# pyranha-labs/hypergrep

Measured on AMD Instinct MI355X. Metric: GiB/s scanned (256 patterns, 32 GiB synthetic log per GPU, text resident in HBM), higher is better.
Workload: dtype u8

## Files before the change

hypergrep_amd/build.py:

```python
from __future__ import annotations

import os
import shutil
import subprocess
import sys

PKG = os.path.dirname(os.path.abspath(__file__))
REPO = os.path.dirname(PKG)
CSRC = os.path.join(PKG, "csrc")
LIB_DIR = os.path.join(PKG, "lib")
LIB = os.path.join(LIB_DIR, "libhyperscanner.so")
LIBHS_NAME = "libhs.so.5"
OBJ = os.path.join(REPO, "build", "obj")
EXTRA = os.environ.get("HG_BUILD_DEFINES", "").split()
if os.environ.get("HG_BUILD_OUT"):
    LIB = os.path.abspath(os.environ["HG_BUILD_OUT"])
    LIB_DIR = os.path.dirname(LIB)
    OBJ = LIB + ".obj"
    LIBHS_NAME = os.path.basename(LIB) + ".libhs.so.5"

HIP_SOURCES = ["hg_stream.hip", "hg_kernels.hip", "hg_always_on.hip", "hg_huge.hip", "hg_som.hip", "hg_comb.hip", "hg_invert.hip", "hg_flows.hip", "hg_batch.hip", "hg_engine.hip", "hg_capi.hip", "hg_shim.hip", "hg_hsface.hip"]
CXX_SOURCES = ["hg_compile.cpp"]
HEADERS = ["hg_mem.h", "hg_db.h", "hg_core.h", "hg_post.h", "hg_engine.h", "hg_compile.h", "hg_synth.h", "hg_confirm_dev.h", "hg_sink_dev.h", "hg_tables_dev.h", "hg_som.h", "hg_comb.h", "hg_invert.h", "hg_flows.h", "hg_flow_rules.h", "hg_batch.h", "hg_batch_launch.h"]

# ... 44 lines not shown

def _merge_resources() -> None:
    import json

    table = {}
    for src in KERNEL_SOURCES:
        path = os.path.join(OBJ, src + ".resources.json")
        if os.path.exists(path):
            with open(path, encoding="utf-8") as f:
                table.update(json.load(f))
    with open(os.path.join(LIB_DIR, "kernel_resources.json"), "w", encoding="utf-8") as f:
        json.dump(table, f, indent=1, sort_keys=True)
    for kernel, res in table.items():
        if kernel.startswith("_Z16hg_stream_kernelILi") and "ELb0ELi0E" in kernel and res.get("ScratchSize [bytes/lane]", 0) > 16:
            raise RuntimeError(f"{kernel} uses {res['ScratchSize [bytes/lane]']} bytes of scratch per lane: the streaming hot path must stay in registers")
        if "hg_som_kernel" in kernel and res.get("ScratchSize [bytes/lane]", 0) > 0:
            raise RuntimeError(f"{kernel} uses {res['ScratchSize [bytes/lane]']} bytes of scratch per lane: the start-of-match walks keep their state in registers / LDS")
        if "hg_minlen_kernel" in kernel and res.get("ScratchSize [bytes/lane]", 0) > 0:
            raise RuntimeError(f"{kernel} uses {res['ScratchSize [bytes/lane]']} bytes of scratch per lane: the match-length walks keep their state in registers / LDS")
        if "hg_flow_som_kernel" in kernel and res.get("ScratchSize [bytes/lane]", 0) > 0:
            raise RuntimeError(f"{kernel} uses {res['ScratchSize [bytes/lane]']} bytes of scratch per lane: the stream-mode start-of-match lanes keep their starts in device memory")
        if "hg_block_batch_kernel" in kernel and (res.get("ScratchSize [bytes/lane]", 0) > 0 or res.get("VGPRs Spill", 0) > 0):
            raise RuntimeError(f"{kernel} uses {res['ScratchSize [bytes/lane]']} bytes of scratch per lane, {res['VGPRs Spill']} spilled VGPRs: the batched block scan keeps its automaton state in registers")
        if "hg_comb_kernel" in kernel and res.get("ScratchSize [bytes/lane]", 0) > 0:
            raise RuntimeError(f"{kernel} uses {res['ScratchSize [bytes/lane]']} bytes of scratch per lane: the combination pass keeps its evaluation stack in a register")


def build(verbose: bool = False, force: bool = False) -> str:
    from concurrent.futures import ThreadPoolExecutor

    os.makedirs(OBJ, exist_ok=True)
    os.makedirs(LIB_DIR, exist_ok=True)
    hipcc = _hipcc()
    common_deps = [os.path.join(CSRC, h) for h in HEADERS] + [os.path.join(REPO, "include", "hypergrep_amd.h")]
    objs, jobs = [], []
    for src in HIP_SOURCES + CXX_SOURCES:
        path = os.path.join(CSRC, src)
        if not os.path.exists(path):
            continue
        obj = os.path.join(OBJ, src + ".o")
        objs.append(obj)
        if force or _stale(obj, [path] + common_deps):
            if src.endswith(".hip"):
                cmd = [hipcc, "--offload-arch=gfx950", "-O3", "-std=c++17", "-fPIC", "-Wall", "-Wno-pass-failed"] + EXTRA + ["-c", path, "-o", obj]
            else:
                cmd = ["g++", "-O2", "-std=c++17", "-fPIC", "-Wall", "-Wextra", "-c", path, "-o", obj]
# ... 34 lines not shown
```

hypergrep_amd/csrc/hg_engine.h:

```cpp
#pragma once
#include <hip/hip_runtime.h>

#include <memory>
#include <string>

#include "../../include/hypergrep_amd.h"
#include "hg_compile.h"
#include "hg_core.h"
#include "hg_invert.h"
#include "hg_post.h"

#ifndef HG_STREAM_WG_WAVES
#define HG_STREAM_WG_WAVES 8
#endif
constexpr uint32_t HG_STREAM_WG_WAVES_DEFAULT = HG_STREAM_WG_WAVES;

constexpr uint32_t HG_CONFIRM_SPLIT = 4;
constexpr uint32_t HG_DEFER_SHARDS = 64;

struct HgDeferred {
  uint64_t pos;
  uint32_t pattern;
  uint32_t rank;
};
// ... 196 lines not shown
  HgTileElem *d_agg_ = nullptr;
  HgCand *d_cands_ = nullptr;
  HgDeferred *d_deferred_ = nullptr;
  uint32_t *d_defer_count_ = nullptr;
  HgHit *d_hits_raw_ = nullptr, *d_hits_out_ = nullptr;
  HgHitAux *d_aux_raw_ = nullptr, *d_aux_out_ = nullptr;
  HgHit *d_acc_hits_ = nullptr;
  HgHitAux *d_acc_aux_ = nullptr;
  uint64_t acc_cap_ = 0;
  bool side_bound_ = false;
  uint64_t *d_key_a_ = nullptr, *d_key_b_ = nullptr;
  uint32_t *d_perm_a_ = nullptr, *d_perm_b_ = nullptr;
  uint8_t *d_keep_ = nullptr;
  uint32_t *d_counters_ = nullptr, *d_selected_ = nullptr, *d_seg_count_ = nullptr;
  uint32_t max_segs_ = 0;
  uint32_t *d_pflags_ = nullptr;
  void *d_temp_ = nullptr;
  size_t temp_bytes_ = 0;
  uint32_t *h_counters_ = nullptr;
  HgTileBase *h_final_ = nullptr;
  hipEvent_t ev_[4] = {nullptr, nullptr, nullptr, nullptr};
  static constexpr int kMaxChunks = 64;
  hipStream_t side_stream_ = nullptr;
  hipEvent_t ev_tile_done_ = nullptr;
  hipEvent_t ev_fin_early_ = nullptr;
  hipEvent_t ev_k1_begin_[kMaxChunks] = {}, ev_k1_end_[kMaxChunks] = {}, ev_side_done_[kMaxChunks] = {};
  uint32_t *d_fin_fill_ = nullptr, *d_fin_kept_ = nullptr, *d_fin_total_ = nullptr, *d_fin_big_ = nullptr;
  bool fin_fallback_ = false;
  uint32_t fin_alloc_ = 0;
  uint32_t fin_epoch_ = 0;
  uint64_t fin_expect_hits_ = 0;
  void *d_huge_claim_ = nullptr;
  uint64_t huge_claim_slots_ = 0;
  uint32_t *d_from_ = nullptr;
  uint64_t from_cap_ = 0;
  uint32_t som_max_nw_ = 0;
  uint32_t *d_min_lengths_ = nullptr;
  HgHit *d_minlen_hits_ = nullptr;
  HgHitAux *d_minlen_aux_ = nullptr;
  uint64_t minlen_cap_ = 0;
  uint32_t minlen_max_nw_ = 0;
  HgComb *d_combs_ = nullptr;
  uint32_t *d_comb_words_ = nullptr, *d_comb_feed_ = nullptr;
  uint32_t *d_comb_count_ = nullptr;
  uint64_t *d_comb_pos_ = nullptr;
  uint64_t comb_in_cap_ = 0;
  HgHit *d_comb_hits_ = nullptr;
// ... 15 lines not shown
```

hypergrep_amd/csrc/hg_engine.hip:

```cpp
#include <algorithm>
#include <array>
#include <cstdio>
#include <cstdlib>
#include <cstring>
#include <memory>

#include "hg_engine.h"
#include "hg_mem.h"

#include <rocprim/rocprim.hpp>

bool hg_launch_stream(const HgStreamArgs &a, uint32_t grid, hipStream_t stream);
bool hg_launch_stream_join(const HgStreamArgs &a, uint32_t grid, hipStream_t stream);
int hg_stream_blocks_per_cu(uint32_t filter_log2, uint32_t filter_wide, uint32_t dense);
__global__ void hg_tile_reduce_kernel(const HgTileSum *sums, uint64_t tile_begin, uint64_t tile_end, uint64_t bs1, HgTileElem *agg);
__global__ void hg_tile_spine_kernel(const HgTileElem *agg, uint32_t nblocks, uint64_t bs1, HgTileBase *block_base, HgTileBase *state);
__global__ void hg_tile_apply_kernel(const HgTileSum *sums, uint64_t tile_begin, uint64_t tile_end, uint64_t bs1, const HgTileBase *block_base,
                                     HgTileBase *bases);
__global__ void hg_tile_inner_kernel(const uint8_t *text, HgTileSum *sums, uint64_t tile_begin, uint64_t tile_end, uint64_t bs1);
__global__ void hg_verify_kernel(HgConfirmArgs a);
__global__ void hg_confirm_fast_kernel(HgConfirmArgs a, uint32_t blocks_per_mode);
__global__ void hg_confirm_generic_kernel(HgConfirmArgs a);
__global__ void hg_always_on_kernel(HgConfirmArgs a, uint32_t first, uint32_t last);
__global__ void hg_always_on_fast_kernel(HgConfirmArgs a);
__global__ void hg_always_on_finish_kernel(HgConfirmArgs a);
__global__ void hg_block_mark_kernel(HgConfirmArgs a, uint32_t *pattern_flags);
__global__ void hg_block_scan_kernel(HgConfirmArgs a, const uint32_t *pattern_flags);
__global__ void hg_block_small_kernel(HgDbView db, const uint8_t *h_text, uint32_t length, HgHit *h_out, uint32_t seg_cap, uint32_t *h_counts, uint32_t *d_done,
                                      uint32_t *h_flag, uint32_t seq, uint32_t ppw);
__global__ void hg_reset_kernel(uint32_t *state, uint32_t state_words, HgTileBase *final_state, uint64_t carry_start, uint64_t first_piece, uint32_t *fill, uint32_t nb, uint32_t *defer_count,
                                uint32_t ndefer);
__global__ void hg_fin_sort_small_kernel(const HgHit *hits, uint32_t *idx, const uint32_t *fill, uint32_t b_lo, uint32_t b_hi, uint32_t cap, uint32_t id_bits,
                                         uint32_t to_bits, uint32_t *kept_count, uint32_t *big_list, uint32_t *big_count, uint32_t big_stride);
template <uint32_t LCAP, bool IN_LDS>
__global__ void hg_fin_sort_big_kernel(const HgHit *hits, uint32_t *idx, const uint32_t *fill, const uint32_t *big_list, const uint32_t *big_count, uint32_t cap,
                                       uint32_t id_bits, uint32_t to_bits, uint32_t *kept_count, uint32_t *overflow, uint64_t *scratch_key, uint32_t *scratch_idx);
template <uint32_t THREADS>
__global__ void hg_fin_scan_kernel(uint32_t *kept_count, uint32_t b_lo, uint32_t b_hi, uint32_t *total, const uint32_t *fill, uint32_t cap, uint32_t *part, uint32_t epoch);
__global__ void hg_confirm_literal_kernel(HgConfirmArgs a);
__global__ void hg_verify_lean_kernel(HgConfirmArgs a);
__global__ void hg_fin_gather_kernel(const HgHit *hits, const HgHitAux *aux, const uint32_t *idx, const uint32_t *kept_base, const uint32_t *total, uint32_t b_lo,
                                     uint32_t b_hi, uint32_t cap, HgHit *oh, HgHitAux *oa);
__global__ void hg_key_kernel(const HgHit *hits, const HgHitAux *aux, const HgPattern *patterns, uint32_t n, uint64_t *key, uint32_t *idx);
__global__ void hg_line_key_kernel(const HgHit *hits, const uint32_t *perm, uint32_t n, uint64_t *key);
__global__ void hg_offset_kernel(uint32_t *idx, uint32_t n, uint32_t add);
__global__ void hg_key_packed_kernel(const HgHit *hits, const HgHitAux *aux, const HgPattern *patterns, uint32_t n, uint32_t id_bits, uint32_t to_bits,
                                     uint64_t *key, uint32_t *idx);
__global__ void hg_keep_kernel(const HgHit *hits, const HgHitAux *aux, const uint32_t *perm, const HgPattern *patterns, uint32_t n, uint8_t *keep);
__global__ void hg_scatter_kernel(const HgHit *hits, const HgHitAux *aux, const uint32_t *perm, const uint8_t *keep, const uint32_t *pos, uint32_t n,
                                  HgHit *oh, HgHitAux *oa, uint32_t *count);

size_t hg_huge_lds_bytes(uint32_t nw_max, uint32_t stage_cap);
bool hg_launch_confirm_huge(const HgConfirmArgs &a, uint32_t grid, uint32_t nw_max, uint32_t stage_cap, void *claim, uint32_t claim_mask, hipStream_t stream);
bool hg_launch_always_on_huge(const HgConfirmArgs &a, uint32_t grid, uint32_t nw_max, uint32_t stage_cap, uint32_t first, uint32_t last, hipStream_t stream);
bool hg_launch_block_huge(const HgConfirmArgs &a, uint32_t grid, uint32_t nw_max, uint32_t stage_cap, const uint32_t *pattern_flags, hipStream_t stream);

namespace {
constexpr int TS_BLOCK_TILES = 1024;
constexpr int STREAM_WG_WAVES = HG_STREAM_WG_WAVES;

template <typename T>
hipError_t upload(void **dst, const std::vector<T> &src, const char *name) {
  size_t bytes = std::max<size_t>(src.size() * sizeof(T), 16);
// ... 121 lines not shown
    const HgPattern &p = db.patterns[i];
    if (p.flags & HG_FLAG_SOM_LEFTMOST) som_max_nw_ = std::max(som_max_nw_, p.nw);
    if (!db.min_lengths.empty() && db.min_lengths[i]) minlen_max_nw_ = std::max(minlen_max_nw_, p.nw);
  }
  if (db.comb_pass()) {
    HG_TRY(upload(reinterpret_cast<void **>(&d_combs_), db.combs, "d_combs_"), "upload combinations");
    HG_TRY(upload(reinterpret_cast<void **>(&d_comb_words_), db.comb_words, "d_comb_words_"), "upload combinations");
    HG_TRY(upload(reinterpret_cast<void **>(&d_comb_feed_), db.comb_feed, "d_comb_feed_"), "upload combinations");
  }
  view_.fold_mask = db.fold_mask;
  view_.window_mask = db.window_mask;
  static_assert(HG_CNT_CURSORS == kMaxChunks, "one tile cursor per pipeline chunk");
  HG_TRY(hgmem::dev_alloc(&d_counters_, HG_ST_ALLOC_WORDS * 4, "d_state_"), "alloc state");
  HG_TRY(hipMemset(d_counters_, 0, HG_ST_ALLOC_WORDS * 4), "clear state");
  d_fin_total_ = d_counters_ + HG_ST_FIN_TOTAL;
  d_selected_ = d_counters_ + HG_ST_SELECTED;
  d_final_ = reinterpret_cast<HgTileBase *>(d_counters_ + HG_ST_FINAL);
  HG_TRY(hgmem::dev_alloc(&d_pflags_, db.patterns.size() * 4 + 16, "d_pflags_"), "alloc pattern flags");
  HG_TRY(hgmem::host_alloc(&h_counters_, (HG_CNT_WORDS + 4 + HG_DEFER_SHARDS) * 4, "h_counters_"), "alloc pinned");
  h_final_ = reinterpret_cast<HgTileBase *>(h_counters_ + HG_ST_FINAL);
  for (auto &ev : ev_) HG_TRY(hipEventCreate(&ev), "hipEventCreate");
  HG_TRY(hipStreamCreateWithFlags(&side_stream_, hipStreamNonBlocking), "hipStreamCreate");
  HG_TRY(hipEventCreateWithFlags(&ev_fin_early_, hipEventDisableTiming), "hipEventCreate");
  HG_TRY(hipEventCreateWithFlags(&ev_tile_done_, hipEventDisableTiming), "hipEventCreate");
  return HG_OK;
}

HgScanner::~HgScanner() {
  (void)hipSetDevice(device_);
  void *ptrs[] = {d_patterns_, d_pool_, d_factors_, d_windows_, d_bucket_, d_filter_, d_ext_, d_slow_, d_sums_, d_bases_, d_block_base_,
                  d_agg_, d_cands_, d_hits_raw_, d_hits_out_, d_aux_raw_, d_aux_out_,
                  d_key_a_, d_key_b_, d_perm_a_, d_perm_b_, d_keep_, d_counters_, d_temp_, d_seg_count_, d_pflags_, d_deferred_, d_defer_count_, d_seg_count2_, d_cands2_, d_disc_, d_bucket2_, d_windows2_, d_groups_, d_acc_hits_, d_acc_aux_, d_huge_claim_, d_wtab_, d_from_, d_fin_fill_, d_fin_kept_, d_fin_big_,
                  d_combs_, d_comb_words_, d_comb_feed_, d_comb_count_, d_comb_pos_, d_comb_hits_, d_comb_aux_, d_comb_temp_, d_bounds_,
                  d_min_lengths_, d_minlen_hits_, d_minlen_aux_, d_inv_count_, d_inv_pos_, d_inv_temp_, d_inv_hits_, d_inv_aux_};
  for (void *p : ptrs) hgmem::dev_free(p, "scanner");
  hgmem::host_free(h_counters_, "h_counters_");
  for (auto &ev : ev_)
    if (ev) (void)hipEventDestroy(ev);
  for (int i = 0; i < kMaxChunks; i++) {
    if (ev_k1_begin_[i]) (void)hipEventDestroy(ev_k1_begin_[i]);
    if (ev_k1_end_[i]) (void)hipEventDestroy(ev_k1_end_[i]);
    if (ev_side_done_[i]) (void)hipEventDestroy(ev_side_done_[i]);
  }
  if (side_stream_) (void)hipStreamDestroy(side_stream_);
  if (ev_fin_early_) (void)hipEventDestroy(ev_fin_early_);
  if (ev_tile_done_) (void)hipEventDestroy(ev_tile_done_);
}

int HgScanner::alloc_cands(uint64_t n) {
  n = std::min<uint64_t>(n, 0x7FFFFFF0u);
  HG_TRY(realloc_dev(d_cands_, n, "d_cands_"), "workspace alloc (candidates)");
  HG_TRY(realloc_dev(d_cands2_, n, "d_cands2_"), "workspace alloc (candidates)");
  uint32_t modes = 0;
  for (uint32_t m = 0; m < HG_CONFIRM_MODES; m++) modes += db_->n_confirm_mode[m] ? 1 : 0;
  HG_TRY(realloc_dev(d_deferred_, std::max<uint64_t>(modes, 1) * n, "d_deferred_"), "workspace alloc (deferred)");
  hgmem::dev_free(d_huge_claim_, "d_huge_claim_");
  d_huge_claim_ = nullptr;
  huge_claim_slots_ = 0;
  if (db_->n_confirm_mode[4]) {
    uint64_t slots = 1u << 12;
    while (slots < 2 * n) slots <<= 1;
    HG_TRY(hgmem::dev_alloc(&d_huge_claim_, slots * 8, "d_huge_claim_"), "workspace alloc (claim table)");
    huge_claim_slots_ = slots;
  }
  cand_cap_ = static_cast<uint32_t>(n);
  return HG_OK;
}

int HgScanner::alloc_hits(uint64_t n64) {
// ... 179 lines not shown
      ca.mode_present[m] = (db_->n_confirm_mode[m] && ((mode_mask >> m) & 1u)) ? 1 : 0;
      ca.list_of_mode[m] = db_->n_confirm_mode[m] ? next++ : 0;
      ca.list_spread[m] = std::min<uint32_t>(HG_DEFER_SHARDS, std::max<uint32_t>(1, HG_DEFER_SHARDS / std::max<uint32_t>(1, db_->n_confirm_mode[m])) * defer_spread_boost_);
    }
  }
  return p;
}

int HgScanner::alloc_fin(uint32_t nb, hipStream_t stream) {
  uint32_t want = 1u << 16;
  while (want < nb) want <<= 1;
  fin_alloc_ = 0;
  HG_TRY(realloc_dev(d_fin_fill_, want, "d_fin_fill_"), "alloc finalize buckets");
  HG_TRY(realloc_dev(d_fin_kept_, want, "d_fin_kept_"), "alloc finalize buckets");
  HG_TRY(realloc_dev(d_fin_big_, 2 * static_cast<size_t>(want) + 3 * 128, "d_fin_big_"), "alloc finalize buckets");
  HG_TRY(hipMemsetAsync(d_fin_big_ + 2 * static_cast<size_t>(want), 0, 3 * 128 * 4, stream), "clear scan flags");
  fin_alloc_ = want;
  return HG_OK;
}

int HgScanner::launch_fin(const PassPlan &p, hipStream_t s, uint32_t lo, uint32_t hi, bool beside_stream) {
  if (hi <= lo) return HG_OK;
  const uint32_t nbk = hi - lo, cu = static_cast<uint32_t>(num_cus_), fin_cap = p.fin_cap, id_bits = p.id_bits, to_bits = p.to_bits;
  HG_TRY(hipMemsetAsync(d_fin_total_ + 2, 0, 8, s), "memset work list");
  hipLaunchKernelGGL(hg_fin_sort_small_kernel, dim3(std::min<uint32_t>((nbk + 3) / 4, cu * 8)), dim3(256), 0, s, d_hits_raw_, d_perm_a_, d_fin_fill_, lo, hi, fin_cap, id_bits, to_bits,
                     d_fin_kept_, d_fin_big_, d_fin_total_ + 2, fin_alloc_);
  hipLaunchKernelGGL((hg_fin_sort_big_kernel<HG_FIN_MEDIUM_CAP, true>), dim3(std::min<uint32_t>(nbk, cu * 4)), dim3(256), 0, s, d_hits_raw_, d_perm_a_, d_fin_fill_, d_fin_big_, d_fin_total_ + 2,
                     fin_cap, id_bits, to_bits, d_fin_kept_, d_selected_ + 1, static_cast<uint64_t *>(nullptr), static_cast<uint32_t *>(nullptr));
  const uint32_t big_blocks = std::min<uint32_t>(std::min<uint32_t>(nbk, 64u), hit_cap_ / HG_FIN_BUCKET_CAP);
  if (big_blocks)
    hipLaunchKernelGGL((hg_fin_sort_big_kernel<HG_FIN_BUCKET_CAP, false>), dim3(big_blocks), dim3(256), 0, s, d_hits_raw_, d_perm_a_, d_fin_fill_, d_fin_big_ + fin_alloc_,
                       d_fin_total_ + 3, fin_cap, id_bits, to_bits, d_fin_kept_, d_selected_ + 1, d_key_a_, d_perm_b_);
  const uint32_t scan_blocks = std::max<uint32_t>(1, std::min<uint32_t>(128, (nbk + 8191) / 8192));
  uint32_t *part = d_fin_big_ + 2 * static_cast<size_t>(fin_alloc_);
  const uint32_t epoch = ++fin_epoch_ ? fin_epoch_ : ++fin_epoch_;
  if (beside_stream) hipLaunchKernelGGL(hg_fin_scan_kernel<512u>, dim3(scan_blocks), dim3(512), 0, s, d_fin_kept_, lo, hi, d_fin_total_, d_fin_fill_, fin_cap, part, epoch);
  else hipLaunchKernelGGL(hg_fin_scan_kernel<1024u>, dim3(scan_blocks), dim3(1024), 0, s, d_fin_kept_, lo, hi, d_fin_total_, d_fin_fill_, fin_cap, part, epoch);
  hipLaunchKernelGGL(hg_fin_gather_kernel, dim3(std::min<uint32_t>((nbk + 3) / 4, cu * 8)), dim3(256), 0, s, d_hits_raw_, d_aux_raw_, d_perm_a_, d_fin_kept_, d_fin_total_, lo, hi, fin_cap,
                     d_hits_out_, d_aux_out_);
  HG_TRY(hipGetLastError(), "finalize launch");
  return HG_OK;
}

int HgScanner::launch_stream(PassPlan &p, uint32_t c, HgScanOutput *out) {
  const uint32_t wgs_c = p.wgs_of(c), joiners_c = p.joiners_of(c);
  HgStreamArgs sa = p.sa;
  sa.tile_begin = p.cut[c];
// ... 40 lines not shown
  HgConfirmArgs ca = p.ca;
  ca.tile_begin = t0;
  ca.tile_end = t1;
  uint32_t *seg_count = p.set_of(c) ? d_seg_count2_ : d_seg_count_;
  ca.cands = p.set_of(c) ? d_cands2_ : d_cands_;
  ca.seg_count = seg_count;
  ca.cand_seg_cap = p.cand_seg_cap[c ? 1 : 0];
  ca.join_seg0 = p.wgs_of(c);
  ca.join_seg_cap = ca.cand_seg_cap / 4;
  uint32_t confirm_blocks = 1, always_blocks = 1;
  if (p.block_mode) {
    HG_TRY(hipMemsetAsync(d_pflags_, 0, db_->patterns.size() * 4, side), "memset pattern flags");
    if (p.has_anchored) hipLaunchKernelGGL(hg_block_mark_kernel, dim3(segs_c), dim3(256), 0, side, ca, d_pflags_);
    always_blocks = std::max<uint32_t>(static_cast<uint32_t>((db_->patterns.size() + 255) / 256), std::min<uint32_t>(db_->nhuge, 1024u));
    ca.hit_seg_cap = hit_cap_ / always_blocks;
    hipLaunchKernelGGL(hg_block_scan_kernel, dim3(static_cast<uint32_t>((db_->patterns.size() + 255) / 256)), dim3(256), 0, side, ca, d_pflags_);
    if (db_->nhuge && !hg_launch_block_huge(ca, std::min<uint32_t>(db_->nhuge, 1024u), db_->huge_max_nw, db_->huge_stage_words, d_pflags_, side)) return huge_lds_error();
    HG_TRY(hipGetLastError(), "block-mode launch");
    p.stage_blocks = std::max(confirm_blocks, always_blocks);
    return HG_OK;
  }
  const uint64_t span = t1 - t0;
  const uint32_t nblocks = static_cast<uint32_t>((span + TS_BLOCK_TILES - 1) / TS_BLOCK_TILES);
  if (p.bs1 < HG_TILE_BYTES) {
    uint32_t blocks = static_cast<uint32_t>(std::min<uint64_t>((span + 255) / 256, 4096));
    hipLaunchKernelGGL(hg_tile_inner_kernel, dim3(blocks), dim3(256), 0, side, p.text, d_sums_, t0, t1, p.bs1);
  }
  hipLaunchKernelGGL(hg_tile_reduce_kernel, dim3(nblocks), dim3(256), 0, side, d_sums_, t0, t1, p.bs1, d_agg_);
  hipLaunchKernelGGL(hg_tile_spine_kernel, dim3(1), dim3(256), 0, side, d_agg_, nblocks, p.bs1, d_block_base_, d_final_);
  hipLaunchKernelGGL(hg_tile_apply_kernel, dim3(nblocks), dim3(256), 0, side, d_sums_, t0, t1, p.bs1, d_block_base_, d_bases_);
  HG_TRY(hipGetLastError(), "tile scan launch");
  if (p.piped && c + 1 == p.nchunks) HG_TRY(hipEventRecord(ev_tile_done_, side), "event");
  if (p.has_anchored) {
    const uint32_t verify_blocks = segs_c * HG_CONFIRM_SPLIT;
    uint32_t fast_modes = 0;
    const uint32_t mode_mask = knobs_.confirm_mode_mask;
    for (uint32_t m = 0; m < 3; m++) fast_modes += (db_->n_confirm_mode[m] && ((mode_mask >> m) & 1u)) ? 1 : 0;
    uint32_t per_cu = c + 1 == p.nchunks ? 6 : 3;
    if (knobs_.confirm_blocks_per_cu) per_cu = static_cast<uint32_t>(knobs_.confirm_blocks_per_cu);
    const uint32_t mode_blocks = std::max<uint32_t>(HG_DEFER_SHARDS, static_cast<uint32_t>(num_cus_) * per_cu * (256 / HG_CONFIRM_THREADS));
    const uint32_t huge_blocks = db_->n_confirm_mode[4] ? std::max<uint32_t>(HG_DEFER_SHARDS, static_cast<uint32_t>(num_cus_) * static_cast<uint32_t>(std::max<size_t>(1, std::min<size_t>(8, (160u << 10) / std::max<size_t>(hg_huge_lds_bytes(db_->huge_max_nw, db_->huge_stage_words), 1))))) : 0u;
    confirm_blocks = std::max(std::max(mode_blocks * std::max(fast_modes, 1u), verify_blocks), huge_blocks);
    ca.hit_seg_cap = hit_cap_ / confirm_blocks;
    if (c > 0) HG_TRY(hipMemsetAsync(d_defer_count_, 0, HG_CONFIRM_MODES * HG_DEFER_SHARDS * 4, side), "memset deferred counts");
    if (ca.mode_present[1] || ca.mode_present[2]) hipLaunchKernelGGL(hg_verify_kernel, dim3(verify_blocks), dim3(256), 0, side, ca);
    else hipLaunchKernelGGL(hg_verify_lean_kernel, dim3(verify_blocks), dim3(256), 0, side, ca);
    const bool literal_only_set = ca.mode_present[0] && !ca.mode_present[1] && !ca.mode_present[2];
    if (literal_only_set) {
      hipLaunchKernelGGL(hg_confirm_literal_kernel, dim3(mode_blocks), dim3(256), 0, side, ca);
    } else if (fast_modes) {
      hipLaunchKernelGGL(hg_confirm_fast_kernel, dim3(mode_blocks * fast_modes), dim3(HG_CONFIRM_THREADS), 0, side, ca, mode_blocks);
    }
    if (db_->n_confirm_mode[3]) hipLaunchKernelGGL(hg_confirm_generic_kernel, dim3(mode_blocks), dim3(256), 0, side, ca);
    if (huge_blocks && ((mode_mask >> 4) & 1u)) {
      HG_TRY(hipMemsetAsync(d_huge_claim_, 0, huge_claim_slots_ * 8, side), "memset claim table");
      if (!hg_launch_confirm_huge(ca, huge_blocks, db_->huge_max_nw, db_->huge_stage_words, d_huge_claim_, static_cast<uint32_t>(huge_claim_slots_ - 1), side)) return huge_lds_error();
    }
    HG_TRY(hipGetLastError(), "confirm launch");
  }
  if (!db_->slow.empty()) {
    always_blocks = static_cast<uint32_t>(std::min<uint64_t>((span + 3) / 4, static_cast<uint64_t>(num_cus_) * 8));
    const uint32_t huge_always_blocks = db_->nslow_huge ? static_cast<uint32_t>(std::min<uint64_t>(span, static_cast<uint64_t>(num_cus_) * 16)) : 0u;
    ca.hit_seg_cap = hit_cap_ / std::max(always_blocks, huge_always_blocks);
    const uint32_t nfast = db_->nslow_fast, nhuge = db_->nslow_huge, nall = static_cast<uint32_t>(db_->slow.size()) - nhuge;
    if (nfast) {
      ca.deferred = d_deferred_;
      ca.always_count = seg_count;
      ca.always_list_cap = cand_cap_ / always_blocks;
      hipLaunchKernelGGL(hg_always_on_fast_kernel, dim3(always_blocks), dim3(256), 0, side, ca);
      hipLaunchKernelGGL(hg_always_on_finish_kernel, dim3(always_blocks), dim3(256), 0, side, ca);
    }
    if (nall > nfast) hipLaunchKernelGGL(hg_always_on_kernel, dim3(always_blocks), dim3(256), 0, side, ca, nfast, nall);
    if (nhuge && !hg_launch_always_on_huge(ca, huge_always_blocks, db_->huge_max_nw, db_->huge_stage_words, nall, nall + nhuge, side)) return huge_lds_error();
    always_blocks = std::max(always_blocks, huge_always_blocks);
    HG_TRY(hipGetLastError(), "hg_always_on_kernel launch");
  }
  p.stage_blocks = std::max(confirm_blocks, always_blocks);
  return HG_OK;
}

int HgScanner::finalize_last(PassPlan &p, uint32_t c) {
  bool fin_early = false;
  if (p.piped && c >= 1 && !knobs_.no_early_finalize) {
    const uint32_t lim = p.settled_buckets(c);
    if (lim > p.fin_done) {
      HG_TRY(hipStreamWaitEvent(p.stream, ev_side_done_[c - 1], 0), "stream wait");
      HG_TRY(hipStreamWaitEvent(p.stream, ev_tile_done_, 0), "stream wait");
      if (int rc = launch_fin(p, p.stream, p.fin_done, lim)) return rc;
      HG_TRY(hipEventRecord(ev_fin_early_, p.stream), "event");
      p.fin_done = lim;
      fin_early = true;
    }
  }
  if (fin_early) HG_TRY(hipStreamWaitEvent(p.side, ev_fin_early_, 0), "stream wait");
  return launch_fin(p, p.side, p.fin_done, p.fin_nb);
}

int HgScanner::regrow(const PassPlan &p, uint64_t n_raw) {
  const bool block_mode = p.block_mode, bucketed = p.bucketed;
  const uint64_t cand_need = h_counters_[HG_CNT_CAND_NEED], hit_need = h_counters_[HG_CNT_HIT_NEED];
  const uint64_t defer_need = h_counters_[HG_CNT_DEFER_NEED];
  const bool fin_overflow = bucketed && h_counters_[HG_ST_SELECTED + 1] != 0;
  uint64_t kHitLimit = 1ull << 28;
  if (knobs_.hit_limit) kHitLimit = std::max<uint64_t>(1u << 10, knobs_.hit_limit);
  if (!block_mode && (n_raw > kHitLimit || h_counters_[HG_CNT_HITS_WRAPPED])) return HG_SPLIT;
  if (!(cand_need || defer_need || hit_need || fin_overflow || (!bucketed && n_raw > hit_cap_))) return HG_OK;
  if (cand_need || defer_need) {
    if (defer_need && defer_spread_boost_ < HG_DEFER_SHARDS) defer_spread_boost_ *= 4;
    uint64_t want = std::max<uint64_t>((cand_need + cand_need / 4 + 64) * p.wgs, (defer_need + defer_need / 4 + 64) * HG_DEFER_SHARDS);
    want = std::max<uint64_t>(want, static_cast<uint64_t>(cand_cap_) * 2);
// ... 406 lines not shown
```

hypergrep_amd/csrc/hg_kernels.hip:

```cpp
#include <hip/hip_runtime.h>
#include <cstdlib>

#include "hg_confirm_dev.h"
#include "hg_core.h"
#include "hg_engine.h"
#include "hg_post.h"
#include "hg_sink_dev.h"
#include "hg_tables_dev.h"

namespace {

__device__ __forceinline__ uint32_t wave_inclusive_scan(uint32_t v, uint32_t lane) {
#pragma unroll
  for (int o = 1; o < 64; o <<= 1) {
    uint32_t u = __shfl_up(v, o, 64);
    if (lane >= static_cast<uint32_t>(o)) v += u;
  }
  return v;
}

}

namespace {
constexpr int TS_THREADS = 256;
// ... 311 lines not shown
          const uint32_t slot = slot0 + __builtin_amdgcn_mbcnt_hi(static_cast<uint32_t>(mm >> 32), __builtin_amdgcn_mbcnt_lo(static_cast<uint32_t>(mm), 0u));
          if (slot < a.defer_shard_cap) a.deferred[(static_cast<uint64_t>(a.list_of_mode[m]) * HG_DEFER_SHARDS + shard) * a.defer_shard_cap + slot] = HgDeferred{pos, tag, o_rank};
          else atomicMax(&a.counters[HG_CNT_DEFER_NEED], slot + 1);
        }
      }
    }
  }
  if (STAGED) verify_stage_flush(a, s_stage);
#ifdef HG_PROFILE_CONFIRM
  if (lane == 0) a.tmp_hits[(6u << 20) + 65536u + blockIdx.x * 4u + wave] = HgHit{pf_t0, static_cast<uint32_t>(wall_clock64() - pf_t0), pf_rounds | (pf_pairs << 8)};
#endif
}
#ifndef HG_VERIFY_WAVES
#define HG_VERIFY_WAVES 4
#endif
#ifndef HG_LITERAL_WAVES
#define HG_LITERAL_WAVES 3
#endif
__global__ __launch_bounds__(256) __attribute__((amdgpu_waves_per_eu(HG_VERIFY_WAVES, HG_VERIFY_WAVES))) void hg_verify_kernel(HgConfirmArgs a) {
  __shared__ VerifyStage s_stage;
  verify_body<true>(a, &s_stage);
}
__global__ __launch_bounds__(256) __attribute__((amdgpu_waves_per_eu(HG_VERIFY_WAVES, HG_VERIFY_WAVES))) void hg_verify_lean_kernel(HgConfirmArgs a) { verify_body<false>(a, nullptr); }

template <int MODE>
__device__ __forceinline__ void confirm_body(const HgConfirmArgs &a, uint32_t vblock, uint32_t vgrid) {
  __shared__ uint32_t s_n, s_base;
  if (threadIdx.x == 0) s_n = 0;
  __syncthreads();
  const uint64_t seg0 = static_cast<uint64_t>(blockIdx.x) * a.hit_seg_cap;
  const HitSink sink{a.tmp_hits + seg0, a.tmp_aux + seg0, a.hit_seg_cap, &s_n};
  const uint32_t shard = vblock % HG_DEFER_SHARDS, peer = vblock / HG_DEFER_SHARDS, peers = (vgrid + HG_DEFER_SHARDS - 1 - shard) / HG_DEFER_SHARDS;
  const HgDeferred *dlist = a.deferred + (static_cast<uint64_t>(a.list_of_mode[MODE]) * HG_DEFER_SHARDS + shard) * a.defer_shard_cap;
  uint32_t n = a.defer_count[MODE * HG_DEFER_SHARDS + shard];
  if (n > a.defer_shard_cap) n = a.defer_shard_cap;
  for (uint32_t i = peer * blockDim.x + threadIdx.x; i < n; i += peers * blockDim.x) {
    const HgDeferred d = dlist[i];
    const uint32_t pattern = d.pattern & (HG_MAX_PATTERNS - 1u);
    const HgPattern &p = a.db.patterns[pattern];
    const uint32_t id = p.id;
    const bool single = MODE != 3 || p.single != 0;
    auto emit = [&](uint64_t line_no, uint32_t to, uint64_t start, uint32_t len) { sink.push(a, line_no, id, to, start, len, pattern, single); };
    if (MODE == 0) hgdev::confirm_literal(a.text, a.nbytes, a.sums, a.bases, a.bs1, d.pos, d.rank, d.pos - (d.pattern >> 24), p.max_len, emit);
    else hg_confirm(a.db, a.text, a.nbytes, a.sums, a.bases, a.bs1, d.pos, pattern, d.rank, emit);
  }
  flush_hits(a, &s_n, &s_base);
// ... 79 lines not shown
        const uint32_t lead = p.lit_lead;
        if (MODE == 1) {
          hgdev::confirm_simple(a.text, a.nbytes, a.sums, a.bases, a.bs1, d.pos, d.rank, fs, lead, p.init_word, p.acc_all, tab + CT_REACH, tab + CT_FOLLOW, emit);
        } else if (nw == 1) {
          hgdev::confirm_ctx<1>(a.text, a.nbytes, a.sums, a.bases, a.bs1, d.pos, d.rank, fs, lead, tab + CT_REACH, tab + CT_FOLLOW, tab + CT_INIT, tab + CT_AMASK,
                                    tab + CT_ACC, emit);
        } else {
          hgdev::confirm_ctx<2>(a.text, a.nbytes, a.sums, a.bases, a.bs1, d.pos, d.rank, fs, lead, tab + CT_REACH, tab + CT_FOLLOW, tab + CT_INIT, tab + CT_AMASK,
                                    tab + CT_ACC, emit);
        }
      }
      __builtin_amdgcn_wave_barrier();
#ifdef HG_PROFILE_CONFIRM
      { const uint64_t n = wall_clock64(); pf_run += n - pf_t; pf_t = n; }
#endif
    }
  }
#ifdef HG_PROFILE_CONFIRM
  if (lane == 0) a.tmp_hits[(6u << 20) + 32768u + blockIdx.x * (HG_CONFIRM_THREADS / 64) + wave] = HgHit{pf_load | (pf_stage << 32), static_cast<uint32_t>(pf_run), pf_pats | (MODE << 28)};
#endif
  flush_hits(a, &s_n, &s_base);
}

#ifdef HG_CONFIRM_WAVES
__attribute__((amdgpu_waves_per_eu(HG_CONFIRM_WAVES, HG_CONFIRM_WAVES)))
#endif
__global__ __launch_bounds__(HG_CONFIRM_THREADS) void hg_confirm_fast_kernel(HgConfirmArgs a, uint32_t blocks_per_mode) {
  uint32_t nmodes = 0;
  for (uint32_t m = 0; m < 3; m++) nmodes += a.mode_present[m] ? 1u : 0u;
  if (nmodes == 0) return;
  const uint32_t k = nmodes - 1u - blockIdx.x / blocks_per_mode, vblock = blockIdx.x % blocks_per_mode;
  uint32_t mode = 0, seen = 0;
  for (uint32_t m = 0; m < 3; m++)
    if (a.mode_present[m] && seen++ == k) mode = m;
  __shared__ __attribute__((aligned(16))) uint32_t s_tab[(HG_CONFIRM_THREADS / 64) * CT_WORDS];
#ifdef HG_PROFILE_CONFIRM
  const uint64_t t0 = wall_clock64();
#endif
  if (mode == 0) confirm_body<0>(a, vblock, blocks_per_mode);
  else if (mode == 1) confirm_tables_body<1>(a, vblock, blocks_per_mode, s_tab);
  else confirm_tables_body<2>(a, vblock, blocks_per_mode, s_tab);
#ifdef HG_PROFILE_CONFIRM
  if ((threadIdx.x & 63u) == 0) {
    const uint64_t t1 = wall_clock64();
    const uint32_t w = blockIdx.x * (HG_CONFIRM_THREADS / 64) + (threadIdx.x >> 6);
    a.tmp_hits[(6u << 20) + w] = HgHit{t0, static_cast<uint32_t>(t1 - t0), mode | (vblock << 4)};
  }
#endif
}
__global__ __launch_bounds__(256) void hg_confirm_generic_kernel(HgConfirmArgs a) { confirm_body<3>(a, blockIdx.x, gridDim.x); }
__attribute__((amdgpu_waves_per_eu(HG_LITERAL_WAVES, HG_LITERAL_WAVES)))
__global__ __launch_bounds__(256) void hg_confirm_literal_kernel(HgConfirmArgs a) { confirm_body<0>(a, blockIdx.x, gridDim.x); }

__global__ __launch_bounds__(256) void hg_block_mark_kernel(HgConfirmArgs a, uint32_t *pattern_flags) {
  const HgCand *cseg = a.cands + static_cast<uint64_t>(blockIdx.x) * a.cand_seg_cap;
  const uint32_t n = a.seg_count[blockIdx.x];
  for (uint32_t i = threadIdx.x; i < n; i += blockDim.x) {
    const HgCand c = cseg[i];
    hg_verify_window(a.db, a.text, a.nbytes, c.pos, c.word, [&](uint32_t pattern, uint64_t, uint32_t) { pattern_flags[pattern] = 1; });
  }
}

__global__ __launch_bounds__(256) void hg_block_scan_kernel(HgConfirmArgs a, const uint32_t *pattern_flags) {
  __shared__ uint32_t s_n, s_base;
  if (threadIdx.x == 0) s_n = 0;
  __syncthreads();
  const uint64_t seg0 = static_cast<uint64_t>(blockIdx.x) * a.hit_seg_cap;
  const HitSink sink{a.tmp_hits + seg0, a.tmp_aux + seg0, a.hit_seg_cap, &s_n};
  for (uint32_t p = blockIdx.x * blockDim.x + threadIdx.x; p < a.db.npatterns; p += gridDim.x * blockDim.x) {
    const HgPattern &pat = a.db.patterns[p];
    if (pat.tier == 0 && !pattern_flags[p]) continue;
    if (pat.tier == HG_TIER_COMB) continue;
    if (pat.nw > HG_MAX_W) continue;
    hg_nfa_scan(a.db.pool, pat, a.text, a.nbytes,
                [&](uint32_t to) { sink.push(a, 0, pat.id, to, 0, static_cast<uint32_t>(a.nbytes), p, pat.single != 0); });
// ... 262 lines not shown
      while (__hip_atomic_load(&part[3 * p + 2], __ATOMIC_ACQUIRE, __HIP_MEMORY_SCOPE_AGENT) != epoch) __builtin_amdgcn_s_sleep(2);
      before += __hip_atomic_load(&part[3 * p], __ATOMIC_RELAXED, __HIP_MEMORY_SCOPE_AGENT);
      before_raw += __hip_atomic_load(&part[3 * p + 1], __ATOMIC_RELAXED, __HIP_MEMORY_SCOPE_AGENT);
    }
    before = wave_inclusive_scan(before, lane);
    before_raw = wave_inclusive_scan(before_raw, lane);
    if (lane == 63) {
      s_base[0] = before;
      s_base[1] = before_raw;
    }
  }
  __syncthreads();
  run += carry + s_base[0];
  for (uint32_t i0 = w_lo; i0 < w_hi; i0 += 64) {
    const uint32_t i = i0 + lane;
    const uint32_t c = i < w_hi ? kept_count[i] : 0u;
    const uint32_t incl = wave_inclusive_scan(c, lane);
    if (i < w_hi) kept_count[i] = run + incl - c;
    run += __builtin_amdgcn_readlane(incl, 63);
  }
  if (blockIdx.x == gridDim.x - 1 && threadIdx.x == 0) {
    total[0] = carry + s_base[0] + all;
    total[1] = carry_raw + s_base[1] + all_raw;
  }
}
template __global__ void hg_fin_scan_kernel<512u>(uint32_t *, uint32_t, uint32_t, uint32_t *, const uint32_t *, uint32_t, uint32_t *, uint32_t);
template __global__ void hg_fin_scan_kernel<1024u>(uint32_t *, uint32_t, uint32_t, uint32_t *, const uint32_t *, uint32_t, uint32_t *, uint32_t);
__global__ void hg_fin_gather_kernel(const HgHit *hits, const HgHitAux *aux, const uint32_t *idx, const uint32_t *kept_base, const uint32_t *total, uint32_t b_lo,
                                     uint32_t b_hi, uint32_t cap, HgHit *oh, HgHitAux *oa) {
  const uint32_t lane = threadIdx.x & 63u, wave = (blockIdx.x * blockDim.x + threadIdx.x) >> 6, waves = (gridDim.x * blockDim.x) >> 6;
  auto base_of = [&](uint32_t b) { return b < b_hi ? kept_base[b] : *total; };
  uint32_t b = b_lo + wave;
  uint32_t k0_next = b < b_hi ? kept_base[b] : 0u, k1_next = b < b_hi ? base_of(b + 1) : 0u;
  uint32_t src_next = (b < b_hi && lane < cap) ? idx[b * cap + lane] : 0u;
  for (; b < b_hi; b += waves) {
    const uint32_t k0 = k0_next, n = k1_next - k0, b0 = b * cap;
    const uint32_t src0 = src_next;
    const uint32_t bn = b + waves;
    k0_next = bn < b_hi ? kept_base[bn] : 0u;
    k1_next = bn < b_hi ? base_of(bn + 1) : 0u;
    src_next = (bn < b_hi && lane < cap) ? idx[bn * cap + lane] : 0u;
    for (uint32_t i = lane; i < n; i += 64) {
      const uint32_t src = i < 64 ? src0 : idx[b0 + i];
      HgHit h = hits[src];
      h.to &= ~HG_HIT_SINGLE_BIT;
      h.line_no &= (1ull << HG_HIT_REL_SHIFT) - 1ull;
// ... 43 lines not shown
```

Measured before the change: 5035.

## Fork tail chunk tile scan and verify onto separate streams, add tail kernel variants

```diff
diff --git a/hypergrep_amd/build.py b/hypergrep_amd/build.py
--- a/hypergrep_amd/build.py
+++ b/hypergrep_amd/build.py
@@ -90,6 +90,8 @@
             raise RuntimeError(f"{kernel} uses {res['ScratchSize [bytes/lane]']} bytes of scratch per lane: the stream-mode start-of-match lanes keep their starts in device memory")
         if "hg_block_batch_kernel" in kernel and (res.get("ScratchSize [bytes/lane]", 0) > 0 or res.get("VGPRs Spill", 0) > 0):
             raise RuntimeError(f"{kernel} uses {res['ScratchSize [bytes/lane]']} bytes of scratch per lane, {res['VGPRs Spill']} spilled VGPRs: the batched block scan keeps its automaton state in registers")
+        if "_tail_kernel" in kernel and (res.get("ScratchSize [bytes/lane]", 0) > 0 or res.get("VGPRs Spill", 0) > 0):
+            raise RuntimeError(f"{kernel} uses {res['ScratchSize [bytes/lane]']} bytes of scratch per lane, {res['VGPRs Spill']} spilled VGPRs: a tail instantiation of a side pass trades registers for resident waves only as far as it spills nothing")
         if "hg_comb_kernel" in kernel and res.get("ScratchSize [bytes/lane]", 0) > 0:
             raise RuntimeError(f"{kernel} uses {res['ScratchSize [bytes/lane]']} bytes of scratch per lane: the combination pass keeps its evaluation stack in a register")
 
diff --git a/hypergrep_amd/csrc/hg_engine.h b/hypergrep_amd/csrc/hg_engine.h
--- a/hypergrep_amd/csrc/hg_engine.h
+++ b/hypergrep_amd/csrc/hg_engine.h
@@ -242,7 +242,7 @@
   hipEvent_t ev_[4] = {nullptr, nullptr, nullptr, nullptr};
   static constexpr int kMaxChunks = 64;
   hipStream_t side_stream_ = nullptr;
-  hipEvent_t ev_tile_done_ = nullptr;
+  hipEvent_t ev_tail_fork_ = nullptr, ev_tail_join_ = nullptr;
   hipEvent_t ev_fin_early_ = nullptr;
   hipEvent_t ev_k1_begin_[kMaxChunks] = {}, ev_k1_end_[kMaxChunks] = {}, ev_side_done_[kMaxChunks] = {};
   uint32_t *d_fin_fill_ = nullptr, *d_fin_kept_ = nullptr, *d_fin_total_ = nullptr, *d_fin_big_ = nullptr;
diff --git a/hypergrep_amd/csrc/hg_engine.hip b/hypergrep_amd/csrc/hg_engine.hip
--- a/hypergrep_amd/csrc/hg_engine.hip
+++ b/hypergrep_amd/csrc/hg_engine.hip
@@ -39,6 +39,10 @@
 __global__ void hg_fin_scan_kernel(uint32_t *kept_count, uint32_t b_lo, uint32_t b_hi, uint32_t *total, const uint32_t *fill, uint32_t cap, uint32_t *part, uint32_t epoch);
 __global__ void hg_confirm_literal_kernel(HgConfirmArgs a);
 __global__ void hg_verify_lean_kernel(HgConfirmArgs a);
+__global__ void hg_verify_tail_kernel(HgConfirmArgs a);
+__global__ void hg_verify_lean_tail_kernel(HgConfirmArgs a);
+__global__ void hg_confirm_fast_tail_kernel(HgConfirmArgs a, uint32_t blocks_per_mode);
+__global__ void hg_confirm_literal_tail_kernel(HgConfirmArgs a);
 __global__ void hg_fin_gather_kernel(const HgHit *hits, const HgHitAux *aux, const uint32_t *idx, const uint32_t *kept_base, const uint32_t *total, uint32_t b_lo,
                                      uint32_t b_hi, uint32_t cap, HgHit *oh, HgHitAux *oa);
 __global__ void hg_key_kernel(const HgHit *hits, const HgHitAux *aux, const HgPattern *patterns, uint32_t n, uint64_t *key, uint32_t *idx);
@@ -206,7 +210,8 @@
   for (auto &ev : ev_) HG_TRY(hipEventCreate(&ev), "hipEventCreate");
   HG_TRY(hipStreamCreateWithFlags(&side_stream_, hipStreamNonBlocking), "hipStreamCreate");
   HG_TRY(hipEventCreateWithFlags(&ev_fin_early_, hipEventDisableTiming), "hipEventCreate");
-  HG_TRY(hipEventCreateWithFlags(&ev_tile_done_, hipEventDisableTiming), "hipEventCreate");
+  HG_TRY(hipEventCreateWithFlags(&ev_tail_fork_, hipEventDisableTiming), "hipEventCreate");
+  HG_TRY(hipEventCreateWithFlags(&ev_tail_join_, hipEventDisableTiming), "hipEventCreate");
   return HG_OK;
 }
 
@@ -228,7 +233,8 @@
   }
   if (side_stream_) (void)hipStreamDestroy(side_stream_);
   if (ev_fin_early_) (void)hipEventDestroy(ev_fin_early_);
-  if (ev_tile_done_) (void)hipEventDestroy(ev_tile_done_);
+  if (ev_tail_fork_) (void)hipEventDestroy(ev_tail_fork_);
+  if (ev_tail_join_) (void)hipEventDestroy(ev_tail_join_);
 }
 
 int HgScanner::alloc_cands(uint64_t n) {
@@ -454,7 +460,6 @@
 int HgScanner::launch_fin(const PassPlan &p, hipStream_t s, uint32_t lo, uint32_t hi, bool beside_stream) {
   if (hi <= lo) return HG_OK;
   const uint32_t nbk = hi - lo, cu = static_cast<uint32_t>(num_cus_), fin_cap = p.fin_cap, id_bits = p.id_bits, to_bits = p.to_bits;
-  HG_TRY(hipMemsetAsync(d_fin_total_ + 2, 0, 8, s), "memset work list");
   hipLaunchKernelGGL(hg_fin_sort_small_kernel, dim3(std::min<uint32_t>((nbk + 3) / 4, cu * 8)), dim3(256), 0, s, d_hits_raw_, d_perm_a_, d_fin_fill_, lo, hi, fin_cap, id_bits, to_bits,
                      d_fin_kept_, d_fin_big_, d_fin_total_ + 2, fin_alloc_);
   hipLaunchKernelGGL((hg_fin_sort_big_kernel<HG_FIN_MEDIUM_CAP, true>), dim3(std::min<uint32_t>(nbk, cu * 4)), dim3(256), 0, s, d_hits_raw_, d_perm_a_, d_fin_fill_, d_fin_big_, d_fin_total_ + 2,
@@ -541,34 +546,45 @@
   }
   const uint64_t span = t1 - t0;
   const uint32_t nblocks = static_cast<uint32_t>((span + TS_BLOCK_TILES - 1) / TS_BLOCK_TILES);
+  const bool tail = c + 1 == p.nchunks, fork = tail && p.has_anchored;
+  const hipStream_t tile_stream = fork ? p.stream : side, verify_stream = fork ? side_stream_ : side;
+  if (fork) {
+    HG_TRY(hipEventRecord(ev_tail_fork_, side), "event");
+    HG_TRY(hipStreamWaitEvent(p.piped ? p.stream : side_stream_, ev_tail_fork_, 0), "stream wait");
+  }
   if (p.bs1 < HG_TILE_BYTES) {
     uint32_t blocks = static_cast<uint32_t>(std::min<uint64_t>((span + 255) / 256, 4096));
-    hipLaunchKernelGGL(hg_tile_inner_kernel, dim3(blocks), dim3(256), 0, side, p.text, d_sums_, t0, t1, p.bs1);
-  }
-  hipLaunchKernelGGL(hg_tile_reduce_kernel, dim3(nblocks), dim3(256), 0, side, d_sums_, t0, t1, p.bs1, d_agg_);
-  hipLaunchKernelGGL(hg_tile_spine_kernel, dim3(1), dim3(256), 0, side, d_agg_, nblocks, p.bs1, d_block_base_, d_final_);
-  hipLaunchKernelGGL(hg_tile_apply_kernel, dim3(nblocks), dim3(256), 0, side, d_sums_, t0, t1, p.bs1, d_block_base_, d_bases_);
+    hipLaunchKernelGGL(hg_tile_inner_kernel, dim3(blocks), dim3(256), 0, tile_stream, p.text, d_sums_, t0, t1, p.bs1);
+  }
+  hipLaunchKernelGGL(hg_tile_reduce_kernel, dim3(nblocks), dim3(256), 0, tile_stream, d_sums_, t0, t1, p.bs1, d_agg_);
+  hipLaunchKernelGGL(hg_tile_spine_kernel, dim3(1), dim3(256), 0, tile_stream, d_agg_, nblocks, p.bs1, d_block_base_, d_final_);
+  hipLaunchKernelGGL(hg_tile_apply_kernel, dim3(nblocks), dim3(256), 0, tile_stream, d_sums_, t0, t1, p.bs1, d_block_base_, d_bases_);
   HG_TRY(hipGetLastError(), "tile scan launch");
-  if (p.piped && c + 1 == p.nchunks) HG_TRY(hipEventRecord(ev_tile_done_, side), "event");
+  if (tail && p.piped) HG_TRY(hipEventRecord(ev_tail_join_, tile_stream), "event");
   if (p.has_anchored) {
     const uint32_t verify_blocks = segs_c * HG_CONFIRM_SPLIT;
     uint32_t fast_modes = 0;
     const uint32_t mode_mask = knobs_.confirm_mode_mask;
     for (uint32_t m = 0; m < 3; m++) fast_modes += (db_->n_confirm_mode[m] && ((mode_mask >> m) & 1u)) ? 1 : 0;
-    uint32_t per_cu = c + 1 == p.nchunks ? 6 : 3;
+    uint32_t per_cu = tail ? 6 : 3;
     if (knobs_.confirm_blocks_per_cu) per_cu = static_cast<uint32_t>(knobs_.confirm_blocks_per_cu);
     const uint32_t mode_blocks = std::max<uint32_t>(HG_DEFER_SHARDS, static_cast<uint32_t>(num_cus_) * per_cu * (256 / HG_CONFIRM_THREADS));
     const uint32_t huge_blocks = db_->n_confirm_mode[4] ? std::max<uint32_t>(HG_DEFER_SHARDS, static_cast<uint32_t>(num_cus_) * static_cast<uint32_t>(std::max<size_t>(1, std::min<size_t>(8, (160u << 10) / std::max<size_t>(hg_huge_lds_bytes(db_->huge_max_nw, db_->huge_stage_words), 1))))) : 0u;
     confirm_blocks = std::max(std::max(mode_blocks * std::max(fast_modes, 1u), verify_blocks), huge_blocks);
     ca.hit_seg_cap = hit_cap_ / confirm_blocks;
-    if (c > 0) HG_TRY(hipMemsetAsync(d_defer_count_, 0, HG_CONFIRM_MODES * HG_DEFER_SHARDS * 4, side), "memset deferred counts");
-    if (ca.mode_present[1] || ca.mode_present[2]) hipLaunchKernelGGL(hg_verify_kernel, dim3(verify_blocks), dim3(256), 0, side, ca);
-    else hipLaunchKernelGGL(hg_verify_lean_kernel, dim3(verify_blocks), dim3(256), 0, side, ca);
+    if (c > 0) HG_TRY(hipMemsetAsync(d_defer_count_, 0, HG_CONFIRM_MODES * HG_DEFER_SHARDS * 4, verify_stream), "memset deferred counts");
+    const bool staged = ca.mode_present[1] || ca.mode_present[2];
+    hipLaunchKernelGGL(staged ? (tail ? hg_verify_tail_kernel : hg_verify_kernel) : (tail ? hg_verify_lean_tail_kernel : hg_verify_lean_kernel), dim3(verify_blocks), dim3(256), 0,
+                       verify_stream, ca);
+    if (fork) {
+      if (!p.piped) HG_TRY(hipEventRecord(ev_tail_join_, verify_stream), "event");
+      HG_TRY(hipStreamWaitEvent(side, ev_tail_join_, 0), "stream wait");
+    }
     const bool literal_only_set = ca.mode_present[0] && !ca.mode_present[1] && !ca.mode_present[2];
     if (literal_only_set) {
-      hipLaunchKernelGGL(hg_confirm_literal_kernel, dim3(mode_blocks), dim3(256), 0, side, ca);
+      hipLaunchKernelGGL(tail ? hg_confirm_literal_tail_kernel : hg_confirm_literal_kernel, dim3(mode_blocks), dim3(256), 0, side, ca);
     } else if (fast_modes) {
-      hipLaunchKernelGGL(hg_confirm_fast_kernel, dim3(mode_blocks * fast_modes), dim3(HG_CONFIRM_THREADS), 0, side, ca, mode_blocks);
+      hipLaunchKernelGGL(tail ? hg_confirm_fast_tail_kernel : hg_confirm_fast_kernel, dim3(mode_blocks * fast_modes), dim3(HG_CONFIRM_THREADS), 0, side, ca, mode_blocks);
     }
     if (db_->n_confirm_mode[3]) hipLaunchKernelGGL(hg_confirm_generic_kernel, dim3(mode_blocks), dim3(256), 0, side, ca);
     if (huge_blocks && ((mode_mask >> 4) & 1u)) {
@@ -604,7 +620,7 @@
     const uint32_t lim = p.settled_buckets(c);
     if (lim > p.fin_done) {
       HG_TRY(hipStreamWaitEvent(p.stream, ev_side_done_[c - 1], 0), "stream wait");
-      HG_TRY(hipStreamWaitEvent(p.stream, ev_tile_done_, 0), "stream wait");
+      HG_TRY(hipStreamWaitEvent(p.stream, ev_tail_join_, 0), "stream wait");
       if (int rc = launch_fin(p, p.stream, p.fin_done, lim)) return rc;
       HG_TRY(hipEventRecord(ev_fin_early_, p.stream), "event");
       p.fin_done = lim;
diff --git a/hypergrep_amd/csrc/hg_kernels.hip b/hypergrep_amd/csrc/hg_kernels.hip
--- a/hypergrep_amd/csrc/hg_kernels.hip
+++ b/hypergrep_amd/csrc/hg_kernels.hip
@@ -357,6 +357,15 @@
   verify_body<true>(a, &s_stage);
 }
 __global__ __launch_bounds__(256) __attribute__((amdgpu_waves_per_eu(HG_VERIFY_WAVES, HG_VERIFY_WAVES))) void hg_verify_lean_kernel(HgConfirmArgs a) { verify_body<false>(a, nullptr); }
+#ifndef HG_VERIFY_TAIL_WAVES
+#define HG_VERIFY_TAIL_WAVES 8
+#endif
+#define HG_VERIFY_TAIL_ATTR __attribute__((amdgpu_waves_per_eu(HG_VERIFY_TAIL_WAVES, HG_VERIFY_TAIL_WAVES)))
+__global__ __launch_bounds__(256) HG_VERIFY_TAIL_ATTR void hg_verify_tail_kernel(HgConfirmArgs a) {
+  __shared__ VerifyStage s_stage;
+  verify_body<true>(a, &s_stage);
+}
+__global__ __launch_bounds__(256) HG_VERIFY_TAIL_ATTR void hg_verify_lean_tail_kernel(HgConfirmArgs a) { verify_body<false>(a, nullptr); }
 
 template <int MODE>
 __device__ __forceinline__ void confirm_body(const HgConfirmArgs &a, uint32_t vblock, uint32_t vgrid) {
@@ -482,10 +491,7 @@
   flush_hits(a, &s_n, &s_base);
 }
 
-#ifdef HG_CONFIRM_WAVES
-__attribute__((amdgpu_waves_per_eu(HG_CONFIRM_WAVES, HG_CONFIRM_WAVES)))
-#endif
-__global__ __launch_bounds__(HG_CONFIRM_THREADS) void hg_confirm_fast_kernel(HgConfirmArgs a, uint32_t blocks_per_mode) {
+__device__ __forceinline__ void confirm_fast_body(const HgConfirmArgs &a, uint32_t blocks_per_mode) {
   uint32_t nmodes = 0;
   for (uint32_t m = 0; m < 3; m++) nmodes += a.mode_present[m] ? 1u : 0u;
   if (nmodes == 0) return;
@@ -508,9 +514,15 @@
   }
 #endif
 }
+#ifdef HG_CONFIRM_WAVES
+__attribute__((amdgpu_waves_per_eu(HG_CONFIRM_WAVES, HG_CONFIRM_WAVES)))
+#endif
+__global__ __launch_bounds__(HG_CONFIRM_THREADS) void hg_confirm_fast_kernel(HgConfirmArgs a, uint32_t blocks_per_mode) { confirm_fast_body(a, blocks_per_mode); }
+__global__ __launch_bounds__(HG_CONFIRM_THREADS) void hg_confirm_fast_tail_kernel(HgConfirmArgs a, uint32_t blocks_per_mode) { confirm_fast_body(a, blocks_per_mode); }
 __global__ __launch_bounds__(256) void hg_confirm_generic_kernel(HgConfirmArgs a) { confirm_body<3>(a, blockIdx.x, gridDim.x); }
 __attribute__((amdgpu_waves_per_eu(HG_LITERAL_WAVES, HG_LITERAL_WAVES)))
 __global__ __launch_bounds__(256) void hg_confirm_literal_kernel(HgConfirmArgs a) { confirm_body<0>(a, blockIdx.x, gridDim.x); }
+__global__ __launch_bounds__(256) void hg_confirm_literal_tail_kernel(HgConfirmArgs a) { confirm_body<0>(a, blockIdx.x, gridDim.x); }
 
 __global__ __launch_bounds__(256) void hg_block_mark_kernel(HgConfirmArgs a, uint32_t *pattern_flags) {
   const HgCand *cseg = a.cands + static_cast<uint64_t>(blockIdx.x) * a.cand_seg_cap;
@@ -819,6 +831,7 @@
   if (blockIdx.x == gridDim.x - 1 && threadIdx.x == 0) {
     total[0] = carry + s_base[0] + all;
     total[1] = carry_raw + s_base[1] + all_raw;
+    total[2] = total[3] = 0;
   }
 }
 template __global__ void hg_fin_scan_kernel<512u>(uint32_t *, uint32_t, uint32_t, uint32_t *, const uint32_t *, uint32_t, uint32_t *, uint32_t);
```

Result: no change. 5032 (-0.0%).
